# valida-xyz/valida

Measured on NVIDIA H100. Metric: trace rows/sec proven (Fibonacci), higher is better.
Workload: dtype u32 (BabyBear, 31-bit modular) + ext5

## Files before the change

valida_b200/csrc/ntt.cu:

```cuda
#include "ctx.h"

namespace {

using bb::mul; using bb::add; using bb::sub;

struct PassParams {
    const uint32_t* src; uint32_t* dst;
    uint64_t src_cs, dst_cs;
    uint64_t src_rs, src_gs;
    uint64_t dst_rs, dst_gs;
    uint32_t log_len;
    uint32_t tile;
    uint64_t groups;
    uint32_t inverse;
    uint32_t src_bitrev;
    uint32_t dst_natural;
    uint32_t g_bits;
    uint32_t pre_mode; uint32_t pre_r, pre_g, pre_shift;
    uint32_t post_mode; uint32_t post_shift, post_g, post_k; uint32_t post_scale;
    const uint32_t* root_hi;
    const uint32_t* root3;
    const uint32_t* tab_lo; const uint32_t* tab_hi;
    uint32_t tab_base;
    uint32_t tab_step;
};

__device__ __forceinline__ uint32_t root_pow(const PassParams& p, uint32_t e) {
    const uint32_t a = __ldg(p.root3 + (e & 511)), b = __ldg(p.root3 + 512 + ((e >> 9) & 511)), c = __ldg(p.root3 + 1024 + ((e >> 18) & 511));
    return mul(mul(a, b), c);
}

__device__ __forceinline__ uint32_t pad(uint32_t i) { return i + (i >> 4) + (i >> 9); }

template <int LQ, int RHO>
__device__ __forceinline__ constexpr uint32_t unit_off(uint32_t m) {
    uint32_t o = m << LQ;
    o += (LQ >= 4) ? (m << (LQ >= 4 ? LQ - 4 : 0)) : (m >> (LQ < 4 ? 4 - LQ : 0));
    if (LQ >= 9) o += m << (LQ >= 9 ? LQ - 9 : 0);
    else if (LQ + RHO >= 9) o += m >> (LQ < 9 ? 9 - LQ : 0);
    return o;
}

template <int RHO, int LOG_LEN, int S>
__device__ __forceinline__ void radix_unit(uint32_t* __restrict__ grp, const uint32_t* __restrict__ tw, uint32_t u) {
    constexpr int R = 1 << RHO;
    constexpr int LQ = LOG_LEN - S - RHO;
    constexpr bool IMM = (LQ + RHO >= 4);
    const uint32_t j = u & ((1u << LQ) - 1), blk = u >> LQ;
    const uint32_t base = (blk << (LQ + RHO)) + j;
    uint32_t* const g0 = grp + pad(base);
    uint32_t x[R];
#pragma unroll
    for (int m = 0; m < R; m++) x[m] = IMM ? g0[unit_off<LQ, RHO>(m)] : grp[pad(base + ((uint32_t)m << LQ))];
#pragma unroll
    for (int a = 0; a < RHO; a++) {
        const int half = R >> (a + 1);
        constexpr int E0 = LQ + S;
        const uint32_t tj = j << (S + a);
        const uint32_t* const tw0 = tw + tj + (tj >> 5);
#pragma unroll
        for (int m0 = 0; m0 < R; m0++) {
            if ((m0 & half) == 0) {
                const int m1 = m0 + half, mm = m0 & (half - 1);
                const uint32_t A = x[m0], B = x[m1];
                x[m0] = add(A, B);
                if (a == RHO - 1 && LQ == 0) x[m1] = sub(A, B);
                else {
                    const uint32_t d = A - B + bb::P;
                    uint32_t wv;
                    if (E0 + a >= 5) wv = tw0[((uint32_t)mm << (E0 + a)) + ((uint32_t)mm << (E0 + a >= 5 ? E0 + a - 5 : 0))];
                    else { const uint32_t ti = tj + ((uint32_t)mm << (E0 + a)); wv = tw[ti + (ti >> 5)]; }
                    x[m1] = mul(d, wv);
                }
            }
        }
    }
#pragma unroll
    for (int m = 0; m < R; m++) { if (IMM) g0[unit_off<LQ, RHO>(m)] = x[m]; else grp[pad(base + ((uint32_t)m << LQ))] = x[m]; }
}

template <int RHO, int LOG_LEN, int S>
__device__ __forceinline__ void radix_step(uint32_t* data, const uint32_t* tw, uint32_t T, uint32_t LS, uint32_t tid, uint32_t nt) {
    constexpr int LU = LOG_LEN - RHO;
    const uint32_t total_units = T << LU;
    for (uint32_t w = tid; w < total_units; w += nt) {
        const uint32_t t = w >> LU, u = w & ((1u << LU) - 1);
        radix_unit<RHO, LOG_LEN, S>(data + t * LS, tw, u);
    }
    __syncthreads();
}

template <int LOG_LEN, int S>
__device__ __forceinline__ void all_stages(uint32_t* data, const uint32_t* tw, uint32_t T, uint32_t LS, uint32_t tid, uint32_t nt) {
    if constexpr (LOG_LEN - S >= 4) {
        radix_step<4, LOG_LEN, S>(data, tw, T, LS, tid, nt);
        all_stages<LOG_LEN, S + 4>(data, tw, T, LS, tid, nt);
    } else if constexpr (LOG_LEN - S == 3) {
        radix_step<3, LOG_LEN, S>(data, tw, T, LS, tid, nt);
    } else if constexpr (LOG_LEN - S == 2) {
        radix_step<2, LOG_LEN, S>(data, tw, T, LS, tid, nt);
    } else if constexpr (LOG_LEN - S == 1) {
        radix_step<1, LOG_LEN, S>(data, tw, T, LS, tid, nt);
    }
}

__host__ __device__ constexpr uint32_t cbrev(uint32_t x, int bits) {
    uint32_t r = 0;
    for (int i = 0; i < bits; i++) r |= ((x >> i) & 1u) << (bits - 1 - i);
    return r;
}
template <int LOG_LEN> struct Std {
    static constexpr int LOG_T = 14 - LOG_LEN;
    static constexpr uint32_t T = 1u << (LOG_T > 0 ? LOG_T : 0), L = 1u << LOG_LEN;
    static constexpr uint32_t LS = (L + (L >> 4) + (L >> 9)) | 1;
    static constexpr int LR0 = LOG_LEN - 5;
    static constexpr int LB = LOG_LEN - 9;
};
__device__ __forceinline__ constexpr uint32_t off_b5(uint32_t c) { return c + (c >> 4); }
template <int LR0> __device__ __forceinline__ constexpr uint32_t off_strided(uint32_t k) {
    return (k << LR0) + (LR0 >= 4 ? (k << (LR0 >= 4 ? LR0 - 4 : 0)) : (k >> (LR0 < 4 ? 4 - LR0 : 0))) + (k >> (9 - LR0));
}
template <int LR0> __device__ __forceinline__ uint32_t base_strided(uint32_t r0) { return r0 + (LR0 >= 4 ? (r0 >> 4) : 0u); }
template <int LB> __device__ __forceinline__ uint32_t base_rowrev(uint32_t B) { return (B << LB) + ((B << LB) >> 4) + (B >> (9 - LB)); }
template <int LB> __device__ __forceinline__ constexpr uint32_t off_rowrev(uint32_t c) { return c + (LB >= 4 ? (c >> 4) : 0u); }

template <int LOG_LEN, bool BITREV>
__device__ __forceinline__ void load_strided_std(const PassParams& p, const uint32_t* __restrict__ src, uint32_t* __restrict__ data, uint64_t g0, uint32_t tid) {
    using S = Std<LOG_LEN>;
    const uint32_t tt = tid & (S::T - 1), r0 = tid >> S::LOG_T;
    const uint32_t* g = src + g0 + tt + (uint64_t)r0 * p.src_rs;
    const uint64_t ks = p.src_rs << S::LR0;
    uint32_t* sl;
    if (BITREV) { const uint32_t B = bb::reverse_bits(r0, S::LR0); sl = data + tt * S::LS + (B << 5) + (B << 1) + (B >> 4); }
    else sl = data + tt * S::LS + base_strided<S::LR0>(r0);
#pragma unroll
    for (int kb = 0; kb < 32; kb += 8) {
        uint32_t v[8];
#pragma unroll
        for (int u = 0; u < 8; u++) v[u] = __ldg(g + (uint64_t)(kb + u) * ks);
#pragma unroll
        for (int u = 0; u < 8; u++) sl[BITREV ? off_b5(cbrev(kb + u, 5)) : off_strided<S::LR0>(kb + u)] = v[u];
    }
}
template <int LOG_LEN, bool BITREV>
__device__ __forceinline__ void load_rows_std(const PassParams& p, const uint32_t* __restrict__ src, uint32_t* __restrict__ data, uint64_t g0, uint32_t tid) {
    using S = Std<LOG_LEN>;
    constexpr uint32_t I = 1u << S::LB;
    const uint32_t sb = BITREV ? base_rowrev<S::LB>(bb::reverse_bits(tid, 9)) : tid + (tid >> 4);
#pragma unroll
    for (uint32_t t = 0; t < S::T; t++) {
        const uint32_t* g = src + (g0 + t) * p.src_gs + tid;
        uint32_t* sl = data + t * S::LS + sb;
#pragma unroll
        for (uint32_t kb = 0; kb < I; kb += 8) {
            uint32_t v[8];
#pragma unroll
            for (uint32_t u = 0; u < 8 && kb + u < I; u++) v[u] = __ldg(g + 512 * (kb + u));
#pragma unroll
            for (uint32_t u = 0; u < 8 && kb + u < I; u++) sl[BITREV ? off_rowrev<S::LB>(cbrev(kb + u, S::LB)) : (kb + u) * 545u] = v[u];
        }
    }
}

template <int LOG_LEN>
__device__ __forceinline__ void load_rows_odd_std(const PassParams& p, const uint32_t* __restrict__ src, uint32_t* __restrict__ data, uint64_t g0, uint32_t tid) {
    using S = Std<LOG_LEN>;
    constexpr uint32_t I = 1u << S::LB;
    const uint32_t B = bb::reverse_bits(tid, 9);
    const uint32_t sb = base_rowrev<S::LB>(B);
    const uint32_t step = root_pow(p, p.pre_r << p.pre_shift);
#pragma unroll 8
    for (uint32_t t = 0; t < S::T; t++) {
        const uint32_t g = (uint32_t)g0 + t;
        const uint32_t gval = p.g_bits ? bb::reverse_bits(g, (int)p.g_bits) : g;
        uint32_t m = root_pow(p, (((B << S::LB) * p.pre_r) + gval * p.pre_g) << p.pre_shift);
        const uint32_t* gp = src + (uint64_t)g * p.src_gs + tid;
        uint32_t* sl = data + t * S::LS + sb;
#pragma unroll
        for (uint32_t ib = 0; ib < I; ib += 8) {
            uint32_t v[8];
#pragma unroll
            for (uint32_t u = 0; u < 8 && ib + u < I; u++) v[u] = __ldg(gp + 512 * cbrev(ib + u, S::LB));
#pragma unroll
            for (uint32_t u = 0; u < 8 && ib + u < I; u++) { sl[off_rowrev<S::LB>(ib + u)] = mul(v[u], m); m = mul(m, step); }
        }
    }
}

__device__ __forceinline__ void post_begin(const PassParams& p, uint32_t gval, uint32_t k_start, uint32_t k_stride, uint32_t* m, uint32_t* step) {
    if (p.post_mode == 1) {
        uint32_t e0 = (gval * k_start) << p.post_shift, es = (gval * k_stride) << p.post_shift;
        if (p.inverse) { e0 = 0u - e0; es = 0u - es; }
        *m = root_pow(p, e0); *step = root_pow(p, es);
    } else if (p.post_mode == 2) {
        *m = vg_pow_lookup(p.tab_lo, p.tab_hi, gval * p.post_g + k_start * p.post_k);
        *step = p.tab_step;
    } else { *m = p.post_mode == 3 ? p.post_scale : bb::R1; *step = bb::R1; }
}
template <int LOG_LEN, bool NAT>
__device__ __forceinline__ void store_rows_std(const PassParams& p, uint32_t* __restrict__ dst, const uint32_t* __restrict__ data, uint64_t g0, uint32_t tid) {
    using S = Std<LOG_LEN>;
    constexpr uint32_t I = 1u << S::LB;
    const uint32_t B = bb::reverse_bits(tid, 9);
    const uint32_t sb = NAT ? base_rowrev<S::LB>(B) : tid + (tid >> 4);
    const bool running = p.post_mode == 1 || p.post_mode == 2;
#pragma unroll
    for (uint32_t t = 0; t < S::T; t++) {
        const uint32_t g = (uint32_t)g0 + t;
        const uint32_t gval = p.g_bits ? bb::reverse_bits(g, (int)p.g_bits) : g;
        uint32_t m, step;
        post_begin(p, gval, NAT ? tid : (B << S::LB), NAT ? 512u : 1u, &m, &step);
        uint32_t* d = dst + (uint64_t)g * p.dst_gs + tid;
        const uint32_t* sl = data + t * S::LS + sb;
#pragma unroll
        for (uint32_t i = 0; i < I; i++) {
            const uint32_t j = NAT ? i : cbrev(i, S::LB);
            const uint32_t v = sl[NAT ? off_rowrev<S::LB>(cbrev(i, S::LB)) : j * 545u];
            d[512 * j] = p.post_mode ? mul(v, m) : v;
            if (running) m = mul(m, step);
        }
    }
}
template <int LOG_LEN, bool NAT>
__device__ __forceinline__ void store_short_rows_std(const PassParams& p, uint32_t* __restrict__ dst, const uint32_t* __restrict__ data, uint64_t g0, uint32_t tid) {
    using S = Std<LOG_LEN>;
    constexpr uint32_t GPS = 512u >> LOG_LEN;
    const uint32_t pos = tid & (S::L - 1), t0 = tid >> LOG_LEN;
    const uint32_t q = NAT ? bb::reverse_bits(pos, LOG_LEN) : pos;
    uint32_t* d = dst + (g0 + t0) * p.dst_gs + pos;
    const uint64_t ks = p.dst_gs * GPS;
    const uint32_t* sl = data + t0 * S::LS + pad(q);
#pragma unroll
    for (uint32_t kb = 0; kb < 32; kb += 8) {
        uint32_t v[8];
#pragma unroll
        for (uint32_t u = 0; u < 8; u++) v[u] = sl[(kb + u) * GPS * S::LS];
#pragma unroll
        for (uint32_t u = 0; u < 8; u++) d[(uint64_t)(kb + u) * ks] = p.post_mode == 3 ? mul(v[u], p.post_scale) : v[u];
    }
}
template <int LOG_LEN, bool NAT>
__device__ __forceinline__ void store_strided_std(const PassParams& p, uint32_t* __restrict__ dst, const uint32_t* __restrict__ data, uint64_t g0, uint32_t tid) {
    using S = Std<LOG_LEN>;
    const uint32_t tt = tid & (S::T - 1), r0 = tid >> S::LOG_T;
    const uint32_t g = (uint32_t)g0 + tt;
    const uint32_t gval = p.g_bits ? bb::reverse_bits(g, (int)p.g_bits) : g;
    const uint32_t Bq = bb::reverse_bits(r0, S::LR0);
    uint32_t m, step;
    post_begin(p, gval, NAT ? r0 : (Bq << 5), NAT ? (1u << S::LR0) : 1u, &m, &step);
    const bool running = p.post_mode == 1 || p.post_mode == 2;
    uint32_t* d = dst + g + (uint64_t)r0 * p.dst_rs;
    const uint64_t ks = p.dst_rs << S::LR0;
    const uint32_t* sl = data + tt * S::LS + (NAT ? (Bq << 5) + (Bq << 1) + (Bq >> 4) : base_strided<S::LR0>(r0));
#pragma unroll
    for (uint32_t i = 0; i < 32; i++) {
        const uint32_t j = NAT ? i : cbrev(i, 5);
        const uint32_t v = sl[NAT ? off_b5(cbrev(i, 5)) : off_strided<S::LR0>(j)];
        d[(uint64_t)j * ks] = p.post_mode ? mul(v, m) : v;
        if (running) m = mul(m, step);
    }
}

template <int LOG_LEN>
__global__ void __launch_bounds__(512) ntt_pass_kernel(PassParams p) {
    extern __shared__ uint32_t smem[];
    constexpr uint32_t L = 1u << LOG_LEN;
    const uint32_t T = p.tile;
    const uint32_t LS = (L + (L >> 4) + (L >> 9)) | 1;
    uint32_t* tw = smem;
    uint32_t* data = smem + (L >= 2 ? L / 2 + L / 64 + 1 : 1);
    const uint32_t tid = threadIdx.x, nt = blockDim.x;
    const uint64_t col = blockIdx.y;
    const uint64_t g0 = (uint64_t)blockIdx.x * T;
    const uint32_t* src = p.src + col * p.src_cs;
    uint32_t* dst = p.dst + col * p.dst_cs;

    {
        const uint64_t unit = (1ull << VG_LOG_NMAX) >> LOG_LEN;
        for (uint32_t j = tid; j < L / 2; j += nt) {
            uint64_t e = (uint64_t)j * unit;
            if (p.inverse && e) e = (1ull << VG_LOG_NMAX) - e;
            tw[j + (j >> 5)] = __ldg(p.root_hi + (e >> VG_POW_LO_BITS));
        }
    }
    const uint32_t total = L * T;
    const uint32_t log_t = 31 - __clz(T);
    bool std_shape = false, loaded = false;
    if constexpr (LOG_LEN >= 8 && LOG_LEN <= 14) {
        std_shape = (T == Std<LOG_LEN>::T) && nt == 512;
        if constexpr (LOG_LEN >= 9) {
            if (std_shape && p.pre_mode && p.src_bitrev && p.src_rs == 1 && p.src_gs != 1) { load_rows_odd_std<LOG_LEN>(p, src, data, g0, tid); loaded = true; }
        }
        if (std_shape && !p.pre_mode) {
            if constexpr (LOG_LEN <= 12) {
                if (p.src_gs == 1) {
                    if (p.src_bitrev) load_strided_std<LOG_LEN, true>(p, src, data, g0, tid); else load_strided_std<LOG_LEN, false>(p, src, data, g0, tid);
                    loaded = true;
                }
            }
            if constexpr (LOG_LEN >= 9) {
                if (!loaded && p.src_rs == 1 && p.src_gs != 1) {
                    if (p.src_bitrev) load_rows_std<LOG_LEN, true>(p, src, data, g0, tid); else load_rows_std<LOG_LEN, false>(p, src, data, g0, tid);
                    loaded = true;
                }
            }
        }
    }
    if (!loaded) {
        const bool tfast = (p.src_gs == 1);
        const uint32_t log_nt = 31 - __clz(nt);
        if (p.pre_mode && p.src_bitrev && !tfast && L >= 4 * nt) {
            const uint32_t ibits = LOG_LEN - log_nt, I = 1u << ibits;
            const uint32_t r_start = bb::reverse_bits(tid, (int)log_nt) << ibits;
            const uint32_t step = root_pow(p, p.pre_r << p.pre_shift);
            const uint32_t step2 = mul(step, step), step3 = mul(step2, step), step4 = mul(step2, step2);
            for (uint32_t t = 0; t < T; t++) {
                const uint32_t g = (uint32_t)g0 + t;
                const uint32_t gval = p.g_bits ? bb::reverse_bits(g, (int)p.g_bits) : g;
                uint32_t m = root_pow(p, (r_start * p.pre_r + gval * p.pre_g) << p.pre_shift);
                const uint32_t* srow = src + (uint64_t)g * p.src_gs;
                uint32_t* drow = data + t * LS;
                for (uint32_t i = 0; i < I; i += 4) {
                    uint32_t v[4];
#pragma unroll
                    for (int u = 0; u < 4; u++) v[u] = srow[tid + (bb::reverse_bits(i + u, (int)ibits) << log_nt)];
                    drow[pad(r_start + i)] = mul(v[0], m);
                    drow[pad(r_start + i + 1)] = mul(v[1], mul(m, step));
                    drow[pad(r_start + i + 2)] = mul(v[2], mul(m, step2));
                    drow[pad(r_start + i + 3)] = mul(v[3], mul(m, step3));
                    m = mul(m, step4);
                }
            }
        } else
        for (uint32_t idx0 = tid; idx0 < total; idx0 += 4 * nt) {
            uint32_t v[4], tt[4], rr[4];
#pragma unroll
            for (int u = 0; u < 4; u++) {
                const uint32_t idx = idx0 + u * nt;
                if (idx < total) {
                    if (tfast) { tt[u] = idx & (T - 1); rr[u] = idx >> log_t; } else { rr[u] = idx & (L - 1); tt[u] = idx >> LOG_LEN; }
                    v[u] = src[(uint64_t)rr[u] * p.src_rs + (g0 + tt[u]) * p.src_gs];
                }
            }
#pragma unroll
            for (int u = 0; u < 4; u++) {
                const uint32_t idx = idx0 + u * nt;
                if (idx < total) {
                    const uint32_t rnat = p.src_bitrev ? bb::reverse_bits(rr[u], (int)LOG_LEN) : rr[u];
                    uint32_t x = v[u];
                    if (p.pre_mode) {
                        const uint32_t g = (uint32_t)g0 + tt[u];
                        const uint32_t gval = p.g_bits ? bb::reverse_bits(g, (int)p.g_bits) : g;
                        x = mul(x, root_pow(p, (rnat * p.pre_r + gval * p.pre_g) << p.pre_shift));
                    }
                    data[tt[u] * LS + pad(rnat)] = x;
                }
            }
        }
    }
    __syncthreads();
    all_stages<LOG_LEN, 0>(data, tw, T, LS, tid, nt);
    bool stored = false;
    if constexpr (LOG_LEN >= 8 && LOG_LEN <= 14) {
        if (std_shape) {
            if constexpr (LOG_LEN <= 12) {
                if (p.dst_gs == 1) {
                    if (p.dst_natural) store_strided_std<LOG_LEN, true>(p, dst, data, g0, tid); else store_strided_std<LOG_LEN, false>(p, dst, data, g0, tid);
                    stored = true;
                }
            }
            if (!stored && p.dst_rs == 1 && p.dst_gs != 1) {
                if constexpr (LOG_LEN >= 9) {
                    if (p.dst_natural) store_rows_std<LOG_LEN, true>(p, dst, data, g0, tid); else store_rows_std<LOG_LEN, false>(p, dst, data, g0, tid);
                    stored = true;
                } else {
                    if (p.post_mode == 0 || p.post_mode == 3) {
                        if (p.dst_natural) store_short_rows_std<LOG_LEN, true>(p, dst, data, g0, tid); else store_short_rows_std<LOG_LEN, false>(p, dst, data, g0, tid);
                        stored = true;
                    }
                }
            }
        }
    }
    if (!stored) {
        const bool tfast = (p.dst_gs == 1);
        const uint32_t log_nt = 31 - __clz(nt);
        const bool fast = tfast ? (nt >= T && log_nt - log_t <= (uint32_t)LOG_LEN) : (L >= nt);
        if (fast && (p.post_mode == 1 || p.post_mode == 2)) {
            const uint32_t lowbits = tfast ? (log_nt - log_t) : log_nt;
            const uint32_t ibits = LOG_LEN - lowbits, I = 1u << ibits;
            const uint32_t p0 = tfast ? (tid >> log_t) : tid;
            const uint32_t ngroups_here = tfast ? 1u : T;
            for (uint32_t tg = 0; tg < ngroups_here; tg++) {
                const uint32_t t = tfast ? (tid & (T - 1)) : tg;
                const uint32_t g = (uint32_t)g0 + t;
                const uint32_t gval = p.g_bits ? bb::reverse_bits(g, (int)p.g_bits) : g;
                const uint32_t k_start = p.dst_natural ? p0 : (bb::reverse_bits(p0, (int)lowbits) << ibits);
                const uint32_t k_stride = p.dst_natural ? (1u << lowbits) : 1u;
                uint32_t m, step;
                post_begin(p, gval, k_start, k_stride, &m, &step);
                uint32_t* dcol = dst + (uint64_t)g * p.dst_gs;
                const uint32_t* drow = data + t * LS;
                for (uint32_t i = 0; i < I; i++) {
                    const uint32_t j = p.dst_natural ? i : bb::reverse_bits(i, (int)ibits);
                    const uint32_t pos = p0 + (j << lowbits);
                    const uint32_t q = p.dst_natural ? bb::reverse_bits(pos, (int)LOG_LEN) : pos;
                    dcol[(uint64_t)pos * p.dst_rs] = mul(drow[pad(q)], m);
                    m = mul(m, step);
                }
            }
        } else {
            for (uint32_t idx = tid; idx < total; idx += nt) {
                uint32_t t, pos;
                if (tfast) { t = idx & (T - 1); pos = idx >> log_t; } else { pos = idx & (L - 1); t = idx >> LOG_LEN; }
                const uint32_t brp = bb::reverse_bits(pos, (int)LOG_LEN);
                const uint32_t q = p.dst_natural ? brp : pos;
                const uint32_t k = p.dst_natural ? pos : brp;
                uint32_t v = data[t * LS + pad(q)];
                if (p.post_mode) {
                    const uint32_t g = (uint32_t)g0 + t;
                    const uint32_t gval = p.g_bits ? bb::reverse_bits(g, (int)p.g_bits) : g;
                    if (p.post_mode == 1) {
                        uint32_t e = (gval * k) << p.post_shift;
                        if (p.inverse) e = (0u - e);
                        v = mul(v, root_pow(p, e));
                    } else if (p.post_mode == 2) {
                        v = mul(v, vg_pow_lookup(p.tab_lo, p.tab_hi, gval * p.post_g + k * p.post_k));
                    } else {
                        v = mul(v, p.post_scale);
                    }
                }
                dst[(uint64_t)pos * p.dst_rs + (g0 + t) * p.dst_gs] = v;
            }
        }
    }
}

constexpr int LOG_ROW_MAX = 14;
constexpr int LOG_COL_MAX = 12;
constexpr int LOG_TILE_ELEMS = 14;

uint32_t choose_tile(int log_len, uint64_t groups) {
    int lt = LOG_TILE_ELEMS - log_len;
    if (lt < 0) lt = 0;
    if (lt > 6) lt = 6;
    uint32_t t = 1u << lt;
    while (t > groups) t >>= 1;
    return t ? t : 1;
}

int32_t launch_pass(vgpu_ctx* ctx, PassParams p, uint64_t w) {
    p.root_hi = ctx->root_table.hi; p.root3 = ctx->root3;
    const uint32_t L = 1u << p.log_len;
    p.tile = choose_tile((int)p.log_len, p.groups);
    const uint64_t tiles = p.groups / p.tile;
    const uint32_t LS = (L + (L >> 4) + (L >> 9)) | 1;
    const size_t smem = ((L >= 2 ? L / 2 + L / 64 + 1 : 1) + (size_t)p.tile * LS) * sizeof(uint32_t);
    const uint32_t total = L * p.tile;
    uint32_t threads = total / 16 >= 512 ? 512 : (total / 16 >= 32 ? total / 16 : 32);
    if (total >= (1u << 14) && threads > 256) threads = 256 * 2;
    using KernelFn = void (*)(PassParams);
    static const KernelFn kernels[15] = {ntt_pass_kernel<0>, ntt_pass_kernel<1>, ntt_pass_kernel<2>, ntt_pass_kernel<3>, ntt_pass_kernel<4>, ntt_pass_kernel<5>,
                                         ntt_pass_kernel<6>, ntt_pass_kernel<7>, ntt_pass_kernel<8>, ntt_pass_kernel<9>, ntt_pass_kernel<10>, ntt_pass_kernel<11>,
                                         ntt_pass_kernel<12>, ntt_pass_kernel<13>, ntt_pass_kernel<14>};
    if (p.log_len > 14) VG_FAIL(ctx, "ntt: sub-transform 2^%u exceeds the shared-memory tile", p.log_len);
    if (!ctx->ntt_attrs_set) { for (auto k : kernels) VG_CUDA(ctx, cudaFuncSetAttribute(k, cudaFuncAttributeMaxDynamicSharedMemorySize, 200 * 1024)); ctx->ntt_attrs_set = true; }
    if (p.post_mode == 2) {
        uint32_t log_nt = 0; while ((1u << log_nt) < threads) log_nt++;
        uint32_t log_t = 0; while ((1u << log_t) < p.tile) log_t++;
        const bool tfast = (p.dst_gs == 1);
        const uint32_t lowbits = tfast ? (log_nt >= log_t ? log_nt - log_t : 0) : log_nt;
        const uint64_t k_stride = p.dst_natural ? (1ull << lowbits) : 1ull;
        p.tab_step = bb::pow(p.tab_base, k_stride * p.post_k);
    }
    for (uint64_t c0 = 0; c0 < w; c0 += 65535) {
        const uint64_t wc = w - c0 < 65535 ? w - c0 : 65535;
        PassParams q = p;
        q.src = p.src + c0 * p.src_cs; q.dst = p.dst + c0 * p.dst_cs;
        dim3 grid((unsigned)tiles, (unsigned)wc);
        KScope ks(ctx, KC_NTT, 8.0 * (double)(p.groups << p.log_len) * (double)wc);
        kernels[p.log_len]<<<grid, threads, smem, ctx->stream>>>(q);
        VG_LAUNCH_CHECK(ctx);
    }
    return 0;
}

__global__ void repeat_row_kernel(const uint32_t* src, uint64_t src_cs, uint32_t* dst, uint64_t dst_cs, uint64_t H, uint64_t w) {
    uint64_t i = (uint64_t)blockIdx.x * blockDim.x + threadIdx.x;
    if (i >= H * w) return;
    dst[(i / H) * dst_cs + (i % H)] = src[(i / H) * src_cs];
}

__global__ void zero_pad_kernel(const uint32_t* src, uint64_t src_cs, uint32_t* dst, uint64_t dst_cs, uint64_t h, uint64_t H, uint64_t w) {
    uint64_t i = (uint64_t)blockIdx.x * blockDim.x + threadIdx.x;
    if (i >= H * w) return;
    uint64_t c = i / H, r = i % H;
    dst[c * dst_cs + r] = r < h ? src[c * src_cs + r] : 0;
}

void split_col_row(int log_n, int* l_col, int* l_row) {
    if (log_n <= LOG_ROW_MAX) { *l_col = 0; *l_row = log_n; return; }
    int lc = log_n - LOG_ROW_MAX;
    if (lc > LOG_COL_MAX) lc = LOG_COL_MAX;
    if (lc < 4) lc = 4;
    *l_col = lc; *l_row = log_n - lc;
}

}

int32_t vg_ntt_nat2nat(vgpu_ctx* ctx, const uint32_t* src, uint64_t src_cs, uint32_t* dst, uint64_t dst_cs, int log_n, uint64_t w,
                       bool inverse, const PowTable* coset, uint32_t* tmp, uint64_t tmp_cs) {
    const uint64_t n = 1ull << log_n;
    uint32_t ninv = inverse ? bb::inv(bb::to_monty((uint32_t)(n % bb::P))) : bb::R1;
    PassParams p{};
    p.inverse = inverse;
    if (log_n <= LOG_ROW_MAX) {
        p.src = src; p.src_cs = src_cs; p.dst = dst; p.dst_cs = dst_cs;
        p.src_rs = 1; p.src_gs = n; p.dst_rs = 1; p.dst_gs = n;
        p.log_len = log_n; p.groups = 1; p.dst_natural = 1;
        if (coset) { p.post_mode = 2; p.post_g = 0; p.post_k = 1; p.tab_lo = coset->lo; p.tab_hi = coset->hi; p.tab_base = coset->base; }
        else if (inverse) { p.post_mode = 3; p.post_scale = ninv; }
        return launch_pass(ctx, p, w);
    }
    if (log_n > VG_LOG_NMAX) VG_FAIL(ctx, "ntt: 2^%d exceeds BabyBear's two-adicity (2^%d)", log_n, VG_LOG_NMAX);
    const int l1 = (log_n + 1) / 2, l2 = log_n - l1;
    const uint64_t n1 = 1ull << l1, n2 = 1ull << l2;
    p.src = src; p.src_cs = src_cs; p.dst = tmp; p.dst_cs = tmp_cs;
    p.src_rs = n2; p.src_gs = 1; p.dst_rs = 1; p.dst_gs = n1;
    p.log_len = l1; p.groups = n2; p.dst_natural = 1;
    p.post_mode = 1; p.post_shift = VG_LOG_NMAX - log_n;
    VG_TRY(launch_pass(ctx, p, w));
    PassParams q{};
    q.inverse = inverse;
    q.src = tmp; q.src_cs = tmp_cs; q.dst = dst; q.dst_cs = dst_cs;
    q.src_rs = n1; q.src_gs = 1; q.dst_rs = n1; q.dst_gs = 1;
    q.log_len = l2; q.groups = n1; q.dst_natural = 1;
    if (coset) { q.post_mode = 2; q.post_g = 1; q.post_k = (uint32_t)n1; q.tab_lo = coset->lo; q.tab_hi = coset->hi; q.tab_base = coset->base; }
    else if (inverse) { q.post_mode = 3; q.post_scale = ninv; }
    return launch_pass(ctx, q, w);
}

static int32_t intt_nat2bitrev_scaled(vgpu_ctx* ctx, const uint32_t* src, uint64_t src_cs, uint32_t* buf, uint64_t bcs, int log_n, uint64_t w, const PowTable* tab) {
    const uint64_t n = 1ull << log_n;
    int lc, lr;
    split_col_row(log_n, &lc, &lr);
    PassParams p{};
    p.inverse = 1;
    if (lc == 0) {
        p.src = src; p.src_cs = src_cs; p.dst = buf; p.dst_cs = bcs;
        p.src_rs = 1; p.src_gs = n; p.dst_rs = 1; p.dst_gs = n;
        p.log_len = log_n; p.groups = 1; p.dst_natural = 0;
        p.post_mode = 2; p.post_g = 0; p.post_k = 1; p.tab_lo = tab->lo; p.tab_hi = tab->hi; p.tab_base = tab->base;
        return launch_pass(ctx, p, w);
    }
    const uint64_t n1 = 1ull << lc, n2 = 1ull << lr;
    p.src = src; p.src_cs = src_cs; p.dst = buf; p.dst_cs = bcs;
    p.src_rs = n2; p.src_gs = 1; p.dst_rs = n2; p.dst_gs = 1;
    p.log_len = lc; p.groups = n2; p.dst_natural = 0;
    p.post_mode = 1; p.post_shift = VG_LOG_NMAX - log_n;
    VG_TRY(launch_pass(ctx, p, w));
    PassParams q{};
    q.inverse = 1;
    q.src = buf; q.src_cs = bcs; q.dst = buf; q.dst_cs = bcs;
    q.src_rs = 1; q.src_gs = n2; q.dst_rs = 1; q.dst_gs = n2;
    q.log_len = lr; q.groups = n1; q.dst_natural = 0;
    q.g_bits = lc;
    q.post_mode = 2; q.post_g = 1; q.post_k = (uint32_t)n1; q.tab_lo = tab->lo; q.tab_hi = tab->hi; q.tab_base = tab->base;
    return launch_pass(ctx, q, w);
}

static int32_t ntt_bitrev2bitrev(vgpu_ctx* ctx, const uint32_t* coef, uint64_t ccs, uint32_t* dst, uint64_t dst_cs, uint32_t* tmp, uint64_t tcs,
                                 int log_n, uint64_t w, bool odd, bool inverse = false, const PowTable* tab = nullptr) {
    const uint64_t n = 1ull << log_n;
    int lc, lr;
    split_col_row(log_n, &lc, &lr);
    PassParams p{};
    p.inverse = inverse ? 1 : 0;
    if (lc == 0) {
        p.src = coef; p.src_cs = ccs; p.dst = dst; p.dst_cs = dst_cs;
        p.src_rs = 1; p.src_gs = n; p.dst_rs = 1; p.dst_gs = n;
        p.log_len = log_n; p.groups = 1; p.src_bitrev = 1; p.dst_natural = 0;
        if (odd) { p.pre_mode = 1; p.pre_r = 1; p.pre_g = 0; p.pre_shift = VG_LOG_NMAX - (log_n + 1); }
        if (tab) { p.post_mode = 2; p.post_g = 0; p.post_k = 1; p.tab_lo = tab->lo; p.tab_hi = tab->hi; p.tab_base = tab->base; }
        return launch_pass(ctx, p, w);
    }
    const uint64_t n1 = 1ull << lc, n2 = 1ull << lr;
    p.src = coef; p.src_cs = ccs; p.dst = tmp; p.dst_cs = tcs;
    p.src_rs = 1; p.src_gs = n2; p.dst_rs = 1; p.dst_gs = n2;
    p.log_len = lr; p.groups = n1; p.src_bitrev = 1; p.dst_natural = 0;
    p.g_bits = lc;
    if (odd) { p.pre_mode = 1; p.pre_r = (uint32_t)n1; p.pre_g = 1; p.pre_shift = VG_LOG_NMAX - (log_n + 1); }
    p.post_mode = 1; p.post_shift = VG_LOG_NMAX - log_n;
    VG_TRY(launch_pass(ctx, p, w));
    PassParams q{};
    q.inverse = inverse ? 1 : 0;
    q.src = tmp; q.src_cs = tcs; q.dst = dst; q.dst_cs = dst_cs;
    q.src_rs = n2; q.src_gs = 1; q.dst_rs = 1; q.dst_gs = n1;
    q.log_len = lc; q.groups = n2; q.src_bitrev = 1; q.dst_natural = 0;
    if (tab) {
        q.g_bits = lr; q.post_mode = 2; q.post_g = 1; q.post_k = (uint32_t)n2;
        q.tab_lo = tab->lo; q.tab_hi = tab->hi; q.tab_base = tab->base;
    }
    return launch_pass(ctx, q, w);
}

int32_t vg_coset_lde(vgpu_ctx* ctx, const uint32_t* src, uint64_t src_cs, uint64_t h, uint64_t w, uint32_t shift_canonical,
                     uint32_t* dst, uint64_t dst_cs, bool bit_reversed, bool src_bitrev, uint32_t log_blowup) {
    if (src_bitrev && !bit_reversed) VG_FAIL(ctx, "coset_lde: a bit-reversed-row input is only supported with bit-reversed output");
    if (bit_reversed && log_blowup != 1) VG_FAIL(ctx, "coset_lde: committed (bit-reversed) extensions are built for log_blowup = 1 only (FriConfig of basic/src/bin/valida.rs:385-390)");
    int log_n = 0;
    while ((1ull << log_n) < h) log_n++;
    if ((1ull << log_n) != h) VG_FAIL(ctx, "coset_lde: height %llu is not a power of two", (unsigned long long)h);
    if (log_n > LOG_ROW_MAX + LOG_COL_MAX) VG_FAIL(ctx, "coset_lde: heights above 2^%d are not built", LOG_ROW_MAX + LOG_COL_MAX);
    if (log_n + (int)log_blowup > VG_LOG_NMAX) VG_FAIL(ctx, "coset_lde: LDE height 2^%d exceeds BabyBear two-adicity", log_n + (int)log_blowup);
    if (h == 1) {
        const uint64_t H = 1ull << log_blowup;
        repeat_row_kernel<<<(unsigned)((H * w + 127) / 128), 128, 0, ctx->stream>>>(src, src_cs, dst, dst_cs, H, w);
        VG_LAUNCH_CHECK(ctx);
        return 0;
    }
    const PowTable* tab = nullptr;
    uint32_t ninv_canon = bb::from_monty(bb::inv(bb::to_monty((uint32_t)(h % bb::P))));
    VG_TRY(vg_get_shift_table(ctx, shift_canonical, ninv_canon, h, &tab));
    uint64_t batch = (2ull << 30) / (8 * h);
    if (batch < 1) batch = 1;
    if (batch > w) batch = w;
    VgBuf coef_buf(ctx), tmp_buf(ctx);
    VG_TRY(coef_buf.alloc(batch * h * 4));
    VG_TRY(tmp_buf.alloc(batch * h * 4));
    uint32_t *coef = coef_buf.as<uint32_t>(), *tmp = tmp_buf.as<uint32_t>();
    for (uint64_t c0 = 0; c0 < w; c0 += batch) {
        uint64_t wc = w - c0 < batch ? w - c0 : batch;
        if (bit_reversed) {
            VG_TRY(src_bitrev ? ntt_bitrev2bitrev(ctx, src + c0 * src_cs, src_cs, coef, h, tmp, h, log_n, wc, false, true, tab)
                              : intt_nat2bitrev_scaled(ctx, src + c0 * src_cs, src_cs, coef, h, log_n, wc, tab));
            VG_TRY(ntt_bitrev2bitrev(ctx, coef, h, dst + c0 * dst_cs, dst_cs, tmp, h, log_n, wc, false));
            VG_TRY(ntt_bitrev2bitrev(ctx, coef, h, dst + c0 * dst_cs + h, dst_cs, tmp, h, log_n, wc, true));
        } else {
            VG_TRY(vg_ntt_nat2nat(ctx, src + c0 * src_cs, src_cs, coef, h, log_n, wc, true, tab, tmp, h));
            const uint64_t H = h << log_blowup;
            VgBuf padb(ctx), tmp2(ctx);
            VG_TRY(padb.alloc(wc * H * 4));
            VG_TRY(tmp2.alloc(wc * H * 4));
            uint64_t tot = H * wc;
            zero_pad_kernel<<<(unsigned)((tot + 255) / 256), 256, 0, ctx->stream>>>(coef, h, padb.as<uint32_t>(), H, h, H, wc);
            ctx->launches++;
            VG_TRY(vg_ntt_nat2nat(ctx, padb.as<uint32_t>(), H, dst + c0 * dst_cs, dst_cs, log_n + (int)log_blowup, wc, false, nullptr, tmp2.as<uint32_t>(), H));
        }
    }
    return 0;
}
```

Measured before the change: 25.42 million.

## Add persistent row-NTT kernel with L2 prefetch of next tile

For row passes of length 2^13 or 2^14 with 2^14-word tiles, launches a persistent grid sized to resident occupancy. Each block loads its twiddles once and loops over tiles, issuing an L2 prefetch for the next tile before running the butterflies, so global-memory fetch overlaps compute. It also adds a microbenchmark and a profiling script that compare the copy-only and butterfly-only floors. The cost is an extra cudaFuncSetAttribute and occupancy query on every launch, a second __syncthreads per tile, and a prefetch that covers only one line per thread.

```diff
diff --git a/profiles/microbench/ntt_overlap.cu b/profiles/microbench/ntt_overlap.cu
--- /dev/null
+++ b/profiles/microbench/ntt_overlap.cu
@@ -0,0 +1,175 @@
+#include "../../valida_b200/csrc/ntt.cu"
+
+namespace {
+
+enum { NONE = 0, ROWS_ODD, STRIDED, ROWS, SHORT_ROWS };
+int load_path(const PassParams& p) {
+    const uint32_t l = p.log_len;
+    if (l < 8 || l > 14) return NONE;
+    if (l >= 9 && p.pre_mode && p.src_bitrev && p.src_rs == 1 && p.src_gs != 1) return ROWS_ODD;
+    if (p.pre_mode) return NONE;
+    if (l <= 12 && p.src_gs == 1) return STRIDED;
+    if (l >= 9 && p.src_rs == 1 && p.src_gs != 1) return ROWS;
+    return NONE;
+}
+int store_path(const PassParams& p) {
+    const uint32_t l = p.log_len;
+    if (l < 8 || l > 14) return NONE;
+    if (l <= 12 && p.dst_gs == 1) return STRIDED;
+    if (p.dst_rs == 1 && p.dst_gs != 1) {
+        if (l >= 9) return ROWS;
+        if (p.post_mode == 0 || p.post_mode == 3) return SHORT_ROWS;
+    }
+    return NONE;
+}
+
+template <int LOG_LEN>
+__global__ void __launch_bounds__(512) copy_only_kernel(PassParams p, int lpath, int spath) {
+    extern __shared__ uint32_t smem[];
+    constexpr uint32_t L = 1u << LOG_LEN;
+    uint32_t* data = smem + L / 2 + L / 64 + 1;
+    const uint64_t col = blockIdx.y, g0 = (uint64_t)blockIdx.x * Std<LOG_LEN>::T;
+    const uint32_t* src = p.src + col * p.src_cs;
+    uint32_t* dst = p.dst + col * p.dst_cs;
+    const uint32_t tid = threadIdx.x;
+    if constexpr (LOG_LEN >= 9) {
+        if (lpath == ROWS_ODD) load_rows_odd_std<LOG_LEN>(p, src, data, g0, tid);
+        if (lpath == ROWS) { if (p.src_bitrev) load_rows_std<LOG_LEN, true>(p, src, data, g0, tid); else load_rows_std<LOG_LEN, false>(p, src, data, g0, tid); }
+    }
+    if constexpr (LOG_LEN <= 12) {
+        if (lpath == STRIDED) { if (p.src_bitrev) load_strided_std<LOG_LEN, true>(p, src, data, g0, tid); else load_strided_std<LOG_LEN, false>(p, src, data, g0, tid); }
+    }
+    __syncthreads();
+    if constexpr (LOG_LEN <= 12) {
+        if (spath == STRIDED) { if (p.dst_natural) store_strided_std<LOG_LEN, true>(p, dst, data, g0, tid); else store_strided_std<LOG_LEN, false>(p, dst, data, g0, tid); }
+    }
+    if constexpr (LOG_LEN >= 9) {
+        if (spath == ROWS) { if (p.dst_natural) store_rows_std<LOG_LEN, true>(p, dst, data, g0, tid); else store_rows_std<LOG_LEN, false>(p, dst, data, g0, tid); }
+    } else {
+        if (spath == SHORT_ROWS) { if (p.dst_natural) store_short_rows_std<LOG_LEN, true>(p, dst, data, g0, tid); else store_short_rows_std<LOG_LEN, false>(p, dst, data, g0, tid); }
+    }
+}
+
+template <int LOG_LEN>
+__global__ void __launch_bounds__(512) butterflies_only_kernel(uint32_t* out, int reps) {
+    extern __shared__ uint32_t smem[];
+    constexpr uint32_t L = 1u << LOG_LEN;
+    using S = Std<LOG_LEN>;
+    uint32_t* tw = smem;
+    uint32_t* data = smem + L / 2 + L / 64 + 1;
+    for (uint32_t j = threadIdx.x; j < L / 2 + L / 64 + 1; j += 512) tw[j] = (j * 0x9E3779B1u) % bb::P;
+    for (uint32_t j = threadIdx.x; j < S::T * S::LS; j += 512) data[j] = (j * 0x85EBCA6Bu + blockIdx.x) % bb::P;
+    __syncthreads();
+    for (int r = 0; r < reps; r++) all_stages<LOG_LEN, 0>(data, tw, S::T, S::LS, threadIdx.x, 512);
+    if (threadIdx.x == 0) out[blockIdx.x] = data[blockIdx.x % (S::T * S::LS)];
+}
+
+__global__ void fill_kernel(uint32_t* x, uint64_t n) {
+    for (uint64_t i = (uint64_t)blockIdx.x * blockDim.x + threadIdx.x; i < n; i += (uint64_t)gridDim.x * blockDim.x)
+        x[i] = (uint32_t)((i * 0x9E3779B97F4A7C15ull) >> 33) % bb::P;
+}
+
+#define CK(x) do { cudaError_t e_ = (x); if (e_ != cudaSuccess) { fprintf(stderr, "%s: %s\n", #x, cudaGetErrorString(e_)); exit(1); } } while (0)
+
+struct Timer {
+    cudaEvent_t a, b; cudaStream_t s;
+    explicit Timer(cudaStream_t st) : s(st) { CK(cudaEventCreate(&a)); CK(cudaEventCreate(&b)); }
+    template <class F> float ms(F f, int reps) {
+        f(); CK(cudaStreamSynchronize(s));
+        CK(cudaEventRecord(a, s));
+        for (int i = 0; i < reps; i++) f();
+        CK(cudaEventRecord(b, s)); CK(cudaEventSynchronize(b));
+        float t; CK(cudaEventElapsedTime(&t, a, b));
+        return t / reps;
+    }
+};
+
+template <int LOG_LEN>
+void floors(vgpu_ctx* ctx, const PassParams& p, uint64_t w, uint32_t* scratch, float* b_ms, float* c_ms, int reps) {
+    constexpr uint32_t L = 1u << LOG_LEN;
+    using S = Std<LOG_LEN>;
+    const size_t smem = (L / 2 + L / 64 + 1 + (size_t)S::T * S::LS) * 4;
+    CK(cudaFuncSetAttribute(copy_only_kernel<LOG_LEN>, cudaFuncAttributeMaxDynamicSharedMemorySize, (int)smem));
+    CK(cudaFuncSetAttribute(butterflies_only_kernel<LOG_LEN>, cudaFuncAttributeMaxDynamicSharedMemorySize, (int)smem));
+    const uint64_t tiles = p.groups / S::T;
+    Timer t(ctx->stream);
+    const int lpath = load_path(p), spath = store_path(p);
+    if (lpath == NONE || spath == NONE) { fprintf(stderr, "pass of 2^%d has no standard tile movement\n", LOG_LEN); exit(1); }
+    *b_ms = t.ms([&] { copy_only_kernel<LOG_LEN><<<dim3((unsigned)tiles, (unsigned)w), 512, smem, ctx->stream>>>(p, lpath, spath); }, reps);
+    CK(cudaGetLastError());
+    const int loops = 8;
+    *c_ms = t.ms([&] { butterflies_only_kernel<LOG_LEN><<<(unsigned)(tiles * w), 512, smem, ctx->stream>>>(scratch, loops); }, reps) / loops;
+    CK(cudaGetLastError());
+}
+
+}
+
+int main(int argc, char** argv) {
+    const int reps = argc > 1 ? atoi(argv[1]) : 20;
+    vgpu_ctx* ctx = nullptr;
+    if (vgpu_ctx_create(0, nullptr, &ctx) != 0) { fprintf(stderr, "vgpu_ctx_create failed\n"); return 1; }
+    cudaDeviceProp prop; CK(cudaGetDeviceProperties(&prop, 0));
+    printf("{\"device\": \"%s\", \"sms\": %d}\n", prop.name, prop.multiProcessorCount);
+    const struct { const char* chip; int log_n; uint64_t w; } shapes[] = {{"cpu", 22, 51}, {"memory", 24, 14}};
+    for (const auto& sh : shapes) {
+        const uint64_t n = 1ull << sh.log_n;
+        uint32_t *a, *b, *scratch;
+        CK(cudaMalloc(&a, n * sh.w * 4)); CK(cudaMalloc(&b, n * sh.w * 4)); CK(cudaMalloc(&scratch, 1 << 20));
+        fill_kernel<<<1024, 256, 0, ctx->stream>>>(a, n * sh.w);
+        fill_kernel<<<1024, 256, 0, ctx->stream>>>(b, n * sh.w);
+        int lc, lr;
+        split_col_row(sh.log_n, &lc, &lr);
+        const uint64_t n1 = 1ull << lc, n2 = 1ull << lr;
+        const PowTable& tab = ctx->root_table;
+        struct Pass { const char* name; PassParams p; };
+        std::vector<Pass> passes;
+        PassParams p{};
+        p.root_hi = ctx->root_table.hi; p.root3 = ctx->root3;
+        p.src = a; p.src_cs = n; p.dst = b; p.dst_cs = n;
+        {
+            PassParams q = p; q.inverse = 1;
+            q.src_rs = n2; q.src_gs = 1; q.dst_rs = n2; q.dst_gs = 1; q.log_len = lc; q.groups = n2;
+            q.post_mode = 1; q.post_shift = VG_LOG_NMAX - sh.log_n;
+            passes.push_back({"inverse column", q});
+        }
+        {
+            PassParams q = p; q.inverse = 1;
+            q.src_rs = 1; q.src_gs = n2; q.dst_rs = 1; q.dst_gs = n2; q.log_len = lr; q.groups = n1; q.g_bits = lc;
+            q.post_mode = 2; q.post_g = 1; q.post_k = (uint32_t)n1; q.tab_lo = tab.lo; q.tab_hi = tab.hi; q.tab_base = tab.base;
+            passes.push_back({"inverse row", q});
+        }
+        for (int odd = 0; odd < 2; odd++) {
+            PassParams q = p;
+            q.src_rs = 1; q.src_gs = n2; q.dst_rs = 1; q.dst_gs = n2; q.log_len = lr; q.groups = n1; q.src_bitrev = 1; q.g_bits = lc;
+            if (odd) { q.pre_mode = 1; q.pre_r = (uint32_t)n1; q.pre_g = 1; q.pre_shift = VG_LOG_NMAX - (sh.log_n + 1); }
+            q.post_mode = 1; q.post_shift = VG_LOG_NMAX - sh.log_n;
+            passes.push_back({odd ? "odd forward row" : "even forward row", q});
+        }
+        {
+            PassParams q = p;
+            q.src_rs = n2; q.src_gs = 1; q.dst_rs = 1; q.dst_gs = n1; q.log_len = lc; q.groups = n2; q.src_bitrev = 1;
+            passes.push_back({"forward column", q});
+        }
+        for (const auto& ps : passes) {
+            Timer t(ctx->stream);
+            const float a_ms = t.ms([&] { if (launch_pass(ctx, ps.p, sh.w) != 0) { fprintf(stderr, "%s\n", ctx->err.c_str()); exit(1); } }, reps);
+            float b_ms = 0, c_ms = 0;
+            switch (ps.p.log_len) {
+                case 8: floors<8>(ctx, ps.p, sh.w, scratch, &b_ms, &c_ms, reps); break;
+                case 9: floors<9>(ctx, ps.p, sh.w, scratch, &b_ms, &c_ms, reps); break;
+                case 10: floors<10>(ctx, ps.p, sh.w, scratch, &b_ms, &c_ms, reps); break;
+                case 14: floors<14>(ctx, ps.p, sh.w, scratch, &b_ms, &c_ms, reps); break;
+                default: fprintf(stderr, "no floor kernels for 2^%u\n", ps.p.log_len); return 1;
+            }
+            const double gb = 8.0 * (double)n * sh.w / 1e9;
+            printf("{\"chip\": \"%s\", \"log_n\": %d, \"w\": %llu, \"pass\": \"%s\", \"log_len\": %u, \"a_pass_ms\": %.4f, \"b_copy_ms\": %.4f, "
+                   "\"c_butterflies_ms\": %.4f, \"a_gbs\": %.1f, \"b_gbs\": %.1f, \"a_over_b_plus_c\": %.3f, \"a_over_max_b_c\": %.3f}\n",
+                   sh.chip, sh.log_n, (unsigned long long)sh.w, ps.name, ps.p.log_len, a_ms, b_ms, c_ms, gb / (a_ms / 1e3), gb / (b_ms / 1e3),
+                   a_ms / (b_ms + c_ms), a_ms / (b_ms > c_ms ? b_ms : c_ms));
+            fflush(stdout);
+        }
+        CK(cudaFree(a)); CK(cudaFree(b)); CK(cudaFree(scratch));
+    }
+    vgpu_ctx_destroy(ctx);
+    return 0;
+}
diff --git a/profiles/prof_ntt_overlap.py b/profiles/prof_ntt_overlap.py
--- /dev/null
+++ b/profiles/prof_ntt_overlap.py
@@ -0,0 +1,59 @@
+import json
+import os
+import re
+import subprocess
+import sys
+import tempfile
+
+ROOT = os.path.dirname(os.path.dirname(os.path.abspath(__file__)))
+sys.path.insert(0, ROOT)
+from valida_b200 import build as b
+
+
+def card():
+    q = "name,power.limit,clocks.sm,clocks.max.sm"
+    r = subprocess.run(["nvidia-smi", "--query-gpu=" + q, "--format=csv,noheader"], capture_output=True, text=True)
+    return dict(zip(q.split(","), [s.strip() for s in r.stdout.splitlines()[0].split(",")])) if r.returncode == 0 and r.stdout else {}
+
+
+def ptxas_report():
+    with tempfile.TemporaryDirectory() as td:
+        r = subprocess.run([b.NVCC] + b.NVCC_FLAGS + ["-Xptxas", "-v", "-x", "cu", "-c", os.path.join(b.CSRC, "ntt.cu"), "-o", os.path.join(td, "ntt.o")],
+                           capture_output=True, text=True, check=True)
+    out, name = [], None
+    for line in r.stderr.splitlines():
+        m = re.search(r"Compiling entry function '(\S+)'", line)
+        if m:
+            name = subprocess.run(["c++filt"], input=m.group(1), capture_output=True, text=True).stdout.strip()
+            name = re.sub(r"\(anonymous namespace\)::", "", name)
+        elif name and ("spill" in line or "registers" in line):
+            out.append("%s: %s" % (name, line.split("info    :")[-1].strip()))
+    return out
+
+
+def main():
+    reps = int(sys.argv[1]) if len(sys.argv) > 1 and sys.argv[1].isdigit() else 20
+    lib = b.build()
+    with tempfile.TemporaryDirectory() as td:
+        exe = os.path.join(td, "ntt_overlap")
+        subprocess.run([b.NVCC] + b.NVCC_FLAGS + ["-o", exe, os.path.join(ROOT, "profiles", "microbench", "ntt_overlap.cu"),
+                        "-L", os.path.dirname(lib), "-lvalida_b200", "-Xlinker", "-rpath=" + os.path.dirname(lib)], check=True)
+        info = card()
+        proc = subprocess.Popen([exe, str(reps)])
+        clocks = []
+        while proc.poll() is None:
+            c = card().get("clocks.sm", "")
+            if c:
+                clocks.append(int(c.split()[0]))
+        if proc.returncode != 0:
+            raise SystemExit("ntt_overlap failed with exit code %d" % proc.returncode)
+        clocks.sort()
+        info["clocks.sm median while running (MHz)"] = clocks[len(clocks) // 2] if clocks else None
+        print(json.dumps(info), flush=True)
+    if "--ptxas" in sys.argv:
+        for line in ptxas_report():
+            print(line)
+
+
+if __name__ == "__main__":
+    main()
diff --git a/valida_b200/csrc/ntt.cu b/valida_b200/csrc/ntt.cu
--- a/valida_b200/csrc/ntt.cu
+++ b/valida_b200/csrc/ntt.cu
@@ -262,6 +262,47 @@
 }
 
 template <int LOG_LEN>
+__device__ __forceinline__ void fill_twiddles(const PassParams& p, uint32_t* tw, uint32_t tid, uint32_t nt) {
+    constexpr uint32_t L = 1u << LOG_LEN;
+    const uint64_t unit = (1ull << VG_LOG_NMAX) >> LOG_LEN;
+    for (uint32_t j = tid; j < L / 2; j += nt) {
+        uint64_t e = (uint64_t)j * unit;
+        if (p.inverse && e) e = (1ull << VG_LOG_NMAX) - e;
+        tw[j + (j >> 5)] = __ldg(p.root_hi + (e >> VG_POW_LO_BITS));
+    }
+}
+
+template <int LOG_LEN>
+__global__ void __launch_bounds__(512, 2) ntt_rows_persistent_kernel(PassParams p, uint32_t tiles, uint32_t items) {
+    using S = Std<LOG_LEN>;
+    static_assert(S::T * S::L == 512 * 32, "a 2^14-word tile, one 128-byte line per thread");
+    extern __shared__ uint32_t smem[];
+    uint32_t* tw = smem;
+    uint32_t* data = smem + S::L / 2 + S::L / 64 + 1;
+    const uint32_t tid = threadIdx.x;
+    fill_twiddles<LOG_LEN>(p, tw, tid, 512);
+    for (uint32_t it = blockIdx.x; it < items; it += gridDim.x) {
+        const uint32_t col = it / tiles, g0 = (it - col * tiles) * S::T;
+        const uint32_t* src = p.src + (uint64_t)col * p.src_cs;
+        if (p.pre_mode) load_rows_odd_std<LOG_LEN>(p, src, data, g0, tid);
+        else if (p.src_bitrev) load_rows_std<LOG_LEN, true>(p, src, data, g0, tid);
+        else load_rows_std<LOG_LEN, false>(p, src, data, g0, tid);
+        __syncthreads();
+        const uint32_t nx = it + gridDim.x;
+        if (nx < items) {
+            const uint32_t ncol = nx / tiles, ng0 = (nx - ncol * tiles) * S::T;
+            const uint32_t e = tid * 32;
+            const uint32_t* line = p.src + (uint64_t)ncol * p.src_cs + (uint64_t)(ng0 + (e >> LOG_LEN)) * p.src_gs + (e & (S::L - 1));
+            asm volatile("prefetch.global.L2 [%0];" :: "l"(line));
+        }
+        all_stages<LOG_LEN, 0>(data, tw, S::T, S::LS, tid, 512);
+        uint32_t* dst = p.dst + (uint64_t)col * p.dst_cs;
+        if (p.dst_natural) store_rows_std<LOG_LEN, true>(p, dst, data, g0, tid); else store_rows_std<LOG_LEN, false>(p, dst, data, g0, tid);
+        __syncthreads();
+    }
+}
+
+template <int LOG_LEN>
 __global__ void __launch_bounds__(512) ntt_pass_kernel(PassParams p) {
     extern __shared__ uint32_t smem[];
     constexpr uint32_t L = 1u << LOG_LEN;
@@ -275,14 +316,7 @@
     const uint32_t* src = p.src + col * p.src_cs;
     uint32_t* dst = p.dst + col * p.dst_cs;
 
-    {
-        const uint64_t unit = (1ull << VG_LOG_NMAX) >> LOG_LEN;
-        for (uint32_t j = tid; j < L / 2; j += nt) {
-            uint64_t e = (uint64_t)j * unit;
-            if (p.inverse && e) e = (1ull << VG_LOG_NMAX) - e;
-            tw[j + (j >> 5)] = __ldg(p.root_hi + (e >> VG_POW_LO_BITS));
-        }
-    }
+    fill_twiddles<LOG_LEN>(p, tw, tid, nt);
     const uint32_t total = L * T;
     const uint32_t log_t = 31 - __clz(T);
     bool std_shape = false, loaded = false;
@@ -473,13 +507,29 @@
         const uint64_t k_stride = p.dst_natural ? (1ull << lowbits) : 1ull;
         p.tab_step = bb::pow(p.tab_base, k_stride * p.post_k);
     }
+    const bool rows_persistent = p.log_len >= 13 && total == (1u << 14) && threads == 512 && p.src_rs == 1 && p.src_gs != 1 &&
+                                 p.dst_rs == 1 && p.dst_gs != 1 && (!p.pre_mode || p.src_bitrev);
+    using RowFn = void (*)(PassParams, uint32_t, uint32_t);
+    const RowFn rows_kernel = p.log_len == 13 ? ntt_rows_persistent_kernel<13> : ntt_rows_persistent_kernel<14>;
+    uint64_t resident = 0;
+    if (rows_persistent) {
+        VG_CUDA(ctx, cudaFuncSetAttribute(rows_kernel, cudaFuncAttributeMaxDynamicSharedMemorySize, (int)smem));
+        int per_sm = 0;
+        VG_CUDA(ctx, cudaOccupancyMaxActiveBlocksPerMultiprocessor(&per_sm, rows_kernel, 512, smem));
+        resident = (uint64_t)(per_sm > 0 ? per_sm : 1) * (uint64_t)ctx->sm_count;
+    }
     for (uint64_t c0 = 0; c0 < w; c0 += 65535) {
         const uint64_t wc = w - c0 < 65535 ? w - c0 : 65535;
         PassParams q = p;
         q.src = p.src + c0 * p.src_cs; q.dst = p.dst + c0 * p.dst_cs;
-        dim3 grid((unsigned)tiles, (unsigned)wc);
         KScope ks(ctx, KC_NTT, 8.0 * (double)(p.groups << p.log_len) * (double)wc);
-        kernels[p.log_len]<<<grid, threads, smem, ctx->stream>>>(q);
+        if (rows_persistent) {
+            const uint64_t items = tiles * wc;
+            if (items >= (1ull << 31)) VG_FAIL(ctx, "ntt: %llu tiles in one pass", (unsigned long long)items);
+            rows_kernel<<<(unsigned)(items < resident ? items : resident), 512, smem, ctx->stream>>>(q, (uint32_t)tiles, (uint32_t)items);
+        } else {
+            kernels[p.log_len]<<<dim3((unsigned)tiles, (unsigned)wc), threads, smem, ctx->stream>>>(q);
+        }
         VG_LAUNCH_CHECK(ctx);
     }
     return 0;
```

Result: no change. 25.71 million (median of 6 runs) (+1.1%).
